# lazear/sage

Measured on AMD Instinct MI355X. Metric: spectra/sec (whole node), fragment-index search-and-score, human tryptic narrow search, higher is better.
Workload: dtype f32

## Files before the change

### include/sage_hip.h

```cpp
#ifndef SAGE_HIP_H
#define SAGE_HIP_H

#include <stddef.h>
#include <stdint.h>

#ifdef __cplusplus
extern "C" {
#endif

#define SAGE_HIP_ABI_VERSION 6

enum {
    SAGE_HIP_OK = 0,
    SAGE_HIP_ERR_INVALID = 1,
    SAGE_HIP_ERR_NO_DEVICE = 2,
    SAGE_HIP_ERR_HIP = 3,
    SAGE_HIP_ERR_UNSUPPORTED = 4,
    SAGE_HIP_ERR_OOM = 5,
    SAGE_HIP_ERR_INTERNAL = 6
};

enum { SAGE_TOL_PPM = 0, SAGE_TOL_PCT = 1, SAGE_TOL_DA = 2 };
typedef struct SageTolerance {
    int32_t kind;
// ... 143 lines not shown
    const float* precursor_mz;
    const uint8_t* precursor_charge;
    const float* isolation_lo;
    const float* isolation_hi;
    const float* scan_start_time;
    const float* inverse_ion_mobility;
    const uint32_t* file_id;
} SageRawBatch;

int sage_hip_batch_process_upload(SageScorer* scorer, const SageRawBatch* raw, uint64_t take_top_n, int deisotope,
                                  float min_deisotope_mz, uint32_t min_peaks, SageDeviceBatch** out, uint32_t* out_npeaks);
int sage_hip_batch_download(SageDeviceBatch* batch, uint64_t* peak_off, float* masses, float* intensities, float* tic);

int sage_hip_initial_hits(SageScorer* scorer, SageDeviceBatch* batch, uint64_t* packed, uint32_t cap,
                          uint32_t* len, uint64_t* matched_peaks, uint64_t* scored_candidates);

typedef struct SageFragments {
    uint64_t capacity;
    uint64_t* psm_off;
    uint8_t* kinds;
    int32_t* charges;
    int32_t* fragment_ordinals;
    float* intensities;
    float* mz_calculated;
    float* mz_experimental;
} SageFragments;
int sage_hip_annotate_resident(SageScorer* scorer, SageDeviceBatch* batch, const SageFeature* features,
                               const uint32_t* counts, SageFragments* out);

int sage_hip_quick_score_resident(SageScorer* scorer, SageDeviceBatch* batch, int prefilter_low_memory, uint8_t* keep);

typedef struct SageTiming {
    float prelim_ms;
    float rescore_ms;
    float total_ms;
    uint32_t n_launches;
    uint32_t n_wide;
    uint32_t arena_entries;
    uint32_t n_retry;
    float retry_ms;
    uint32_t n_tied;
    uint32_t n_ways;
} SageTiming;
int sage_hip_last_timing(const SageScorer* scorer, SageTiming* out);
int sage_hip_scorer_set_timing_interval(SageScorer* scorer, uint32_t every);

int sage_hip_host_alloc(uint64_t bytes, void** out);
void sage_hip_host_free(void* p);

int sage_hip_debug_phase_cycles(SageScorer* scorer, unsigned long long* out32);
int sage_hip_debug_prune_counters(SageScorer* scorer, unsigned long long* out4);
int sage_hip_debug_filter_counters(SageScorer* scorer, unsigned long long* out4);
int sage_hip_debug_heavy_counters(SageScorer* scorer, unsigned long long* out2);
int sage_hip_debug_handover_route(SageScorer* scorer, uint32_t* out);

typedef struct SageDbLayout {
    uint64_t np, nf;
    uint32_t tile_shift, n_tiles, lut_stride;
    float lut_scale;
    uint32_t tile2_shift, n_tiles2, lut2_stride;
    float lut2_scale;
    uint32_t lut2_words;
    uint32_t pep_lut_bins;
    float pep_lut_inv_w;
    uint32_t ion_lo_bits, ion_hi_bits;
    uint32_t max_ions, max_len;
    uint64_t tm2_pos_len;
} SageDbLayout;
int sage_hip_debug_db_layout(SageDeviceDb* db, SageDbLayout* out);
enum {
    SAGE_DB_IONS = 0, SAGE_DB_ION_OFF = 1, SAGE_DB_PM_OFF = 2, SAGE_DB_PEP_INFO = 3, SAGE_DB_PEP_MONO = 4, SAGE_DB_PEP_LUT = 5,
    SAGE_DB_PM_FRAG = 6, SAGE_DB_TM_FRAG = 7, SAGE_DB_TM2_FRAG = 8, SAGE_DB_TM_LUT = 9, SAGE_DB_TM2_L1 = 10, SAGE_DB_TM2_POS = 11
};
int sage_hip_debug_db_table(SageDeviceDb* db, int table, void* out, uint64_t cap_bytes, uint64_t* out_bytes);

typedef struct SageRescoreInput {
    uint64_t n;
    const SageFeature* features;
    const float* aligned_rt;
    const float* delta_rt_model;
    const float* delta_ims_model;
    SageTolerance precursor_tol;
    const uint32_t* peptide_key;
    uint32_t n_peptide_keys;
    const uint32_t* protein_key;
    uint32_t n_protein_keys;
} SageRescoreInput;

typedef struct SageRescoreOutput {
    float* discriminant_score;
    float* posterior_error;
    float* spectrum_q;
    float* peptide_q;
    float* protein_q;
    uint32_t* order;
    uint64_t passing_spectrum;
    uint64_t passing_peptide;
    uint64_t passing_protein;
    int32_t lda_fitted;
    double coef[20];
    float device_ms;
} SageRescoreOutput;

int sage_hip_rescore(int device, const SageRescoreInput* in, SageRescoreOutput* out);

typedef struct SageRtInput {
// ... 227 lines not shown
```

### sage_amd/_lib.py

```python
import ctypes as C
import os

import numpy as np

from . import build as _build

c_float_p = C.POINTER(C.c_float)
c_u8_p = C.POINTER(C.c_uint8)
c_u32_p = C.POINTER(C.c_uint32)
c_u64_p = C.POINTER(C.c_uint64)


class SageTolerance(C.Structure):
    _fields_ = [("kind", C.c_int32), ("lo", C.c_float), ("hi", C.c_float)]


class SageTheoretical(C.Structure):
    _fields_ = [("peptide_index", C.c_uint32), ("fragment_mz", C.c_float)]


class SageDbParams(C.Structure):
    _fields_ = [
        ("bucket_size", C.c_uint64),
        ("missed_cleavages", C.c_int32),
# ... 263 lines not shown
_lib = None


def lib_path():
    return _build.LIB


def load():
    global _lib
    if _lib is not None:
        return _lib
    if not os.path.exists(_build.LIB) or (os.environ.get("SAGE_HIP_REBUILD") == "1"):
        _build.build(verbose=False)
    lib = C.CDLL(_build.LIB)
    vp = C.c_void_p
    sig = {
        "sage_hip_last_error": (C.c_char_p, []),
        "sage_hip_abi_version": (C.c_int, []),
        "sage_hip_hostdb_build": (C.c_int, [C.c_char_p, C.POINTER(SageDbParams), C.POINTER(vp)]),
        "sage_hip_hostdb_free": (None, [vp]),
        "sage_hip_hostdb_view": (C.c_int, [vp, C.POINTER(SageDbView)]),
        "sage_hip_hostdb_peptide_string": (C.c_uint64, [vp, C.c_uint64, C.c_char_p, C.c_uint64]),
        "sage_hip_hostdb_peptide_proteins": (C.c_uint64, [vp, C.c_uint64, C.c_char_p, C.c_uint64]),
        "sage_hip_hostdb_peptide_info": (C.c_int, [vp, C.c_uint64, c_u32_p, c_u8_p]),
        "sage_hip_process_ms2": (C.c_uint64, [C.c_uint64, C.c_int, C.c_float, c_float_p, c_float_p, C.c_uint64,
                                              C.c_uint8, c_float_p, c_float_p, c_float_p]),
        "sage_hip_device_count": (C.c_int, []),
        "sage_hip_db_create": (C.c_int, [C.POINTER(SageDbView), C.c_int, C.POINTER(vp)]),
        "sage_hip_db_destroy": (None, [vp]),
        "sage_hip_db_device_bytes": (C.c_uint64, [vp]),
        "sage_hip_scorer_create": (C.c_int, [vp, C.POINTER(SageScorerParams), C.POINTER(vp)]),
        "sage_hip_scorer_destroy": (None, [vp]),
        "sage_hip_scorer_clone": (C.c_int, [vp, C.POINTER(vp)]),
        "sage_hip_score_batch": (C.c_int, [vp, C.POINTER(SageSpectrumBatch), vp, c_u32_p]),
        "sage_hip_batch_upload": (C.c_int, [vp, C.POINTER(SageSpectrumBatch), C.POINTER(vp)]),
        "sage_hip_batch_free": (None, [vp]),
        "sage_hip_batch_process_upload": (C.c_int, [vp, C.POINTER(SageRawBatch), C.c_uint64, C.c_int, C.c_float, C.c_uint32,
                                                    C.POINTER(vp), c_u32_p]),
        "sage_hip_batch_download": (C.c_int, [vp, c_u64_p, c_float_p, c_float_p, c_float_p]),
        "sage_hip_batch_upload_kinds": (C.c_int, [vp, C.POINTER(SageSpectrumBatch), c_u8_p, C.POINTER(vp)]),
        "sage_hip_batch_process_upload_kinds": (C.c_int, [vp, C.POINTER(SageRawBatch), c_u8_p, C.c_uint64, C.c_int, C.c_float,
                                                          C.c_uint32, C.POINTER(vp), c_u32_p]),
        "sage_hip_score_batch_kinds": (C.c_int, [vp, C.POINTER(SageSpectrumBatch), c_u8_p, vp, c_u32_p]),
        "sage_hip_score_resident": (C.c_int, [vp, vp, vp, c_u32_p]),
        "sage_hip_initial_hits": (C.c_int, [vp, vp, c_u64_p, C.c_uint32, c_u32_p, c_u64_p, c_u64_p]),
        "sage_hip_last_timing": (C.c_int, [vp, C.POINTER(SageTiming)]),
        "sage_hip_scorer_set_timing_interval": (C.c_int, [vp, C.c_uint32]),
        "sage_hip_annotate_resident": (C.c_int, [vp, vp, vp, c_u32_p, C.POINTER(SageFragments)]),
        "sage_hip_quick_score_resident": (C.c_int, [vp, vp, C.c_int, c_u8_p]),
        "sage_hip_debug_phase_cycles": (C.c_int, [vp, c_u64_p]),
        "sage_hip_debug_prune_counters": (C.c_int, [vp, c_u64_p]),
        "sage_hip_debug_filter_counters": (C.c_int, [vp, c_u64_p]),
        "sage_hip_debug_heavy_counters": (C.c_int, [vp, c_u64_p]),
        "sage_hip_debug_handover_route": (C.c_int, [vp, c_u32_p]),
        "sage_hip_debug_db_layout": (C.c_int, [vp, C.POINTER(SageDbLayout)]),
        "sage_hip_debug_db_table": (C.c_int, [vp, C.c_int, vp, C.c_uint64, c_u64_p]),
        "sage_hip_host_alloc": (C.c_int, [C.c_uint64, C.POINTER(vp)]),
        "sage_hip_host_free": (None, [vp]),
        "sage_hip_rescore": (C.c_int, [C.c_int, C.POINTER(SageRescoreInput), C.POINTER(SageRescoreOutput)]),
        "sage_hip_hostdb_competition_keys": (C.c_int, [vp, c_u32_p, C.c_uint64, c_u32_p, c_u32_p, c_u32_p, c_u32_p]),
        "sage_hip_predict_rt": (C.c_int, [C.c_int, C.POINTER(SageRtInput), C.POINTER(SageRtOutput)]),
        "sage_hip_hostdb_feature_peptides": (C.c_int, [vp, c_u32_p, C.c_uint64, c_u64_p, c_u8_p, c_float_p]),
        "sage_hip_mzml_read": (C.c_int, [C.c_char_p, C.c_uint32, C.c_int, C.POINTER(vp)]),
        "sage_hip_mzml_view": (C.c_int, [vp, C.POINTER(SageRawBatch)]),
        "sage_hip_mzml_check_searchable": (C.c_int, [vp]),
        "sage_hip_mzml_spectrum_id": (C.c_char_p, [vp, C.c_uint64]),
        "sage_hip_mzml_free": (None, [vp]),
        "sage_hip_mzml_read_sn": (C.c_int, [C.c_char_p, C.c_uint32, C.c_int, C.c_int, C.POINTER(vp)]),
        "sage_hip_mzml_ion_injection_time": (C.c_float, [vp, C.c_uint64]),
        "sage_hip_mzml_precursor_ref": (C.c_char_p, [vp, C.c_uint64]),
        "sage_hip_mgf_read": (C.c_int, [C.c_char_p, C.c_uint32, C.POINTER(vp)]),
        "sage_hip_mzml_isolation_kinds": (C.c_int, [vp, c_u8_p]),
        "sage_hip_mzml_charge_zero": (C.c_int, [vp, c_u8_p]),
        "sage_hip_parse_f32": (C.c_int, [C.c_char_p, C.c_uint64, c_float_p]),
        "sage_hip_tmt": (C.c_int, [C.c_int, C.POINTER(SageTmtInput), C.POINTER(SageTmtOutput)]),
        "sage_hip_write_tmt": (C.c_int, [C.c_char_p, C.POINTER(C.c_char_p), C.c_uint32, C.c_uint64, c_u32_p, C.POINTER(C.c_char_p),
                                         c_float_p, c_float_p, C.POINTER(C.c_char_p), C.c_uint32]),
        "sage_hip_write_results": (C.c_int, [C.c_char_p, C.c_int, vp, vp, C.c_uint64, c_u64_p, c_u64_p, C.POINTER(C.c_char_p),
                                             C.c_uint32, C.POINTER(C.c_char_p), C.POINTER(SagePostColumns)]),
        "sage_hip_write_results_grouped": (C.c_int, [C.c_char_p, C.c_int, vp, vp, C.c_uint64, c_u64_p, c_u64_p, C.POINTER(C.c_char_p),
                                                     C.c_uint32, C.POINTER(C.c_char_p), C.POINTER(SagePostColumns),
                                                     C.POINTER(SageGroupColumns)]),
        "sage_hip_protein_groups": (C.c_int, [C.c_int, vp, C.POINTER(SageGroupInput), C.POINTER(SageGroupOutput)]),
        "sage_hip_group_string": (C.c_char_p, [vp, C.c_uint64]),
        "sage_hip_group_strings_free": (None, [vp]),
        "sage_hip_group_graph_build": (C.c_int, [vp, c_u32_p, C.c_uint64, C.POINTER(vp)]),
        "sage_hip_group_graph_view": (C.c_int, [vp, C.POINTER(SageGroupGraphView)]),
        "sage_hip_group_graph_free": (None, [vp]),
        "sage_hip_hostdb_protein_name": (C.c_uint64, [vp, C.c_uint64, C.c_char_p, C.c_uint64]),
        "sage_hip_lfq": (C.c_int, [C.c_int, C.POINTER(SageLfqInput), C.POINTER(SageLfqOutput)]),
        "sage_hip_lfq_im": (C.c_int, [C.c_int, C.POINTER(SageLfqInput), C.POINTER(SageLfqMobility), C.POINTER(SageLfqOutput)]),
        "sage_hip_mzml_mobility": (c_float_p, [vp]),
        "sage_hip_mzml_has_mobility": (C.c_int, [vp, c_u8_p]),
        "sage_hip_write_lfq": (C.c_int, [C.c_char_p, vp, C.POINTER(SageLfqOutput), c_u64_p, C.c_uint64, C.POINTER(C.c_char_p),
                                         C.c_uint32]),
        "sage_hip_fasta_num_targets": (C.c_int, [C.c_char_p, C.POINTER(SageDbParams), c_u64_p]),
        "sage_hip_prefilter_chunk_size": (C.c_int, [C.c_char_p, C.POINTER(SageDbParams), C.c_uint64, c_u64_p]),
        "sage_hip_hostdb_build_chunk": (C.c_int, [C.c_char_p, C.POINTER(SageDbParams), C.c_uint64, C.c_uint64, C.POINTER(vp)]),
        "sage_hip_hostdb_merge_kept": (C.c_int, [C.POINTER(vp), C.POINTER(c_u8_p), C.c_uint32, C.POINTER(SageDbParams),
                                                 C.POINTER(vp)]),
    }
    for name, (res, args) in sig.items():
        fn = getattr(lib, name)
        fn.restype = res
        fn.argtypes = args
    _lib = lib
    return lib


EXPORTED_SYMBOLS = [
    "sage_hip_last_error", "sage_hip_abi_version", "sage_hip_hostdb_build", "sage_hip_hostdb_free",
    "sage_hip_hostdb_view", "sage_hip_hostdb_peptide_string", "sage_hip_hostdb_peptide_proteins",
    "sage_hip_hostdb_peptide_info", "sage_hip_process_ms2", "sage_hip_device_count", "sage_hip_db_create", "sage_hip_db_destroy",
    "sage_hip_db_device_bytes", "sage_hip_scorer_create", "sage_hip_scorer_destroy", "sage_hip_scorer_clone", "sage_hip_score_batch",
    "sage_hip_batch_upload", "sage_hip_batch_free", "sage_hip_batch_process_upload", "sage_hip_batch_download", "sage_hip_score_resident", "sage_hip_initial_hits",
    "sage_hip_last_timing", "sage_hip_scorer_set_timing_interval", "sage_hip_annotate_resident", "sage_hip_quick_score_resident", "sage_hip_debug_phase_cycles", "sage_hip_debug_prune_counters", "sage_hip_debug_filter_counters", "sage_hip_debug_heavy_counters", "sage_hip_debug_handover_route", "sage_hip_debug_db_layout", "sage_hip_debug_db_table", "sage_hip_host_alloc", "sage_hip_host_free",
    "sage_hip_rescore", "sage_hip_hostdb_competition_keys", "sage_hip_fasta_num_targets", "sage_hip_prefilter_chunk_size",
    "sage_hip_hostdb_build_chunk", "sage_hip_hostdb_merge_kept", "sage_hip_predict_rt", "sage_hip_hostdb_feature_peptides",
    "sage_hip_write_results", "sage_hip_mzml_read", "sage_hip_mzml_view", "sage_hip_mzml_check_searchable", "sage_hip_mzml_spectrum_id", "sage_hip_mzml_free",
    "sage_hip_lfq", "sage_hip_write_lfq", "sage_hip_mzml_read_sn", "sage_hip_mzml_ion_injection_time", "sage_hip_mzml_precursor_ref",
    "sage_hip_tmt", "sage_hip_write_tmt", "sage_hip_mgf_read", "sage_hip_mzml_isolation_kinds", "sage_hip_mzml_charge_zero",
    "sage_hip_parse_f32", "sage_hip_batch_upload_kinds", "sage_hip_batch_process_upload_kinds", "sage_hip_score_batch_kinds",
    "sage_hip_lfq_im", "sage_hip_mzml_mobility", "sage_hip_mzml_has_mobility",
    "sage_hip_protein_groups", "sage_hip_group_string", "sage_hip_group_strings_free", "sage_hip_group_graph_build",
    "sage_hip_group_graph_view", "sage_hip_group_graph_free", "sage_hip_hostdb_protein_name", "sage_hip_write_results_grouped",
]


def check(rc):
    if rc != 0:
        msg = load().sage_hip_last_error()
        raise SageHipError(f"libsage_hip status {rc}: {msg.decode() if msg else ''}")


def as_ptr(arr, ctype):
    return arr.ctypes.data_as(C.POINTER(ctype))
```

### sage_amd/csrc/capi.hip

```cpp
#include <hip/hip_runtime.h>
#include <algorithm>
#include <atomic>
#include <cmath>
#include <chrono>
#include <cstring>
#include <memory>
#include <future>
#include <mutex>
#include <string>
#include <vector>

#include "crlog.h"
#include "device_types.h"
#define HIP_FAILED(e, what) fail(status_of(e), std::string(what) + ": " + hipGetErrorString(e))
#include "hip_host.h"
#include "host_db.hpp"

using namespace sagehip;

namespace {

thread_local std::string g_last_error;

int fail(int code, const std::string& msg) {
// ... 2160 lines not shown
    HIP_TRY(hipMemcpy(st.data(), s->ws.status.p, (size_t)n * 4, hipMemcpyDeviceToHost));
    for (uint32_t i = 0; i < n; i++) {
        if (st[i] != ST_OK && st[i] != ST_OK_ORDERED) return fail(SAGE_HIP_ERR_UNSUPPORTED, "spectrum " + std::to_string(i) + ": status " + std::to_string(st[i]));
        for (uint32_t j = 0; j < len[i]; j++) packed[(size_t)i * cap + j] = c[(size_t)i * kmax + j];
        if (matched_peaks) matched_peaks[i] = tot[2 * i];
        if (scored_candidates) scored_candidates[i] = tot[2 * i + 1];
    }
    return SAGE_HIP_OK;
}

int sage_hip_debug_phase_cycles(SageScorer* s, unsigned long long* out32) {
    if (!s || !out32) return fail(SAGE_HIP_ERR_INVALID, "null argument");
    if (!s->dbg.p) return fail(SAGE_HIP_ERR_INVALID, "set SAGE_HIP_PHASE_CLOCKS=1 before creating the scorer");
    std::vector<unsigned long long> all(4096 * 32);
    HIP_TRY(hipMemcpy(all.data(), s->dbg.p, all.size() * 8, hipMemcpyDeviceToHost));
    for (int k = 0; k < 32; k++) out32[k] = 0;
    for (size_t b = 0; b < 4096; b++)
        for (int k = 0; k < 32; k++) out32[k] += all[b * 32 + k];
    return SAGE_HIP_OK;
}

int sage_hip_debug_prune_counters(SageScorer* s, unsigned long long* out4) {
    if (!s || !out4) return fail(SAGE_HIP_ERR_INVALID, "null argument");
    if (!s->dbg.p) return fail(SAGE_HIP_ERR_INVALID, "set SAGE_HIP_PHASE_CLOCKS=1 before creating the scorer");
    std::vector<unsigned long long> all((size_t)DBG_BLOCKS * DBG_PRUNE_WORDS);
    HIP_TRY(hipMemcpy(all.data(), s->dbg.p + (size_t)DBG_BLOCKS * 32, all.size() * 8, hipMemcpyDeviceToHost));
    for (uint32_t k = 0; k < 4; k++) out4[k] = 0;
    for (size_t b = 0; b < DBG_BLOCKS; b++)
        for (uint32_t k = 0; k < 4; k++) out4[k] += all[b * DBG_PRUNE_WORDS + k];
    return SAGE_HIP_OK;
}
int sage_hip_debug_filter_counters(SageScorer* s, unsigned long long* out4) {
    if (!s || !out4) return fail(SAGE_HIP_ERR_INVALID, "null argument");
    if (!s->dbg.p) return fail(SAGE_HIP_ERR_INVALID, "set SAGE_HIP_PHASE_CLOCKS=1 before creating the scorer");
    std::vector<unsigned long long> all((size_t)DBG_BLOCKS * DBG_PRUNE_WORDS);
    HIP_TRY(hipMemcpy(all.data(), s->dbg.p + (size_t)DBG_BLOCKS * 32, all.size() * 8, hipMemcpyDeviceToHost));
    for (uint32_t k = 0; k < 4; k++) out4[k] = 0;
    for (size_t b = 0; b < DBG_BLOCKS; b++)
        for (uint32_t k = 0; k < 4; k++) out4[k] += all[b * DBG_PRUNE_WORDS + 4 + k];
    return SAGE_HIP_OK;
}

int sage_hip_debug_heavy_counters(SageScorer* s, unsigned long long* out2) {
    if (!s || !out2) return fail(SAGE_HIP_ERR_INVALID, "null argument");
    if (!s->dbg.p) return fail(SAGE_HIP_ERR_INVALID, "set SAGE_HIP_PHASE_CLOCKS=1 before creating the scorer");
    std::vector<unsigned long long> all((size_t)DBG_BLOCKS * DBG_PRUNE_WORDS);
    HIP_TRY(hipMemcpy(all.data(), s->dbg.p + (size_t)DBG_BLOCKS * 32, all.size() * 8, hipMemcpyDeviceToHost));
    out2[0] = out2[1] = 0;
    for (size_t b = 0; b < DBG_BLOCKS; b++)
        for (uint32_t k = 0; k < 2; k++) out2[k] += all[b * DBG_PRUNE_WORDS + 8 + k];
    return SAGE_HIP_OK;
}

int sage_hip_debug_handover_route(SageScorer* s, uint32_t* out) {
    if (!s || !out) return fail(SAGE_HIP_ERR_INVALID, "null argument");
    *out = s->last_hand ? 1u : 0u;
    return SAGE_HIP_OK;
}

int sage_hip_debug_db_layout(SageDeviceDb* db, SageDbLayout* out) {
    if (!db || !out) return fail(SAGE_HIP_ERR_INVALID, "null argument");
    const DevDbView& v = db->view;
    std::memset(out, 0, sizeof *out);
    out->np = v.np;
    out->nf = v.nf;
    out->tile_shift = v.tile_shift;
    out->n_tiles = v.n_tiles;
    out->lut_stride = v.lut_stride;
    out->lut_scale = v.lut_scale;
    out->tile2_shift = v.tile2_shift;
    out->n_tiles2 = v.n_tiles2;
    out->lut2_stride = v.lut2_stride;
    out->lut2_scale = v.lut2_scale;
    out->lut2_words = v.lut2_words;
    out->pep_lut_bins = v.pep_lut_bins;
    out->pep_lut_inv_w = v.pep_lut_inv_w;
    out->ion_lo_bits = db->ion_lo_bits;
    out->ion_hi_bits = db->ion_hi_bits;
    out->max_ions = db->max_ions;
    out->max_len = db->max_len;
    out->tm2_pos_len = db->tm2_pos.n;
    return SAGE_HIP_OK;
}

int sage_hip_debug_db_table(SageDeviceDb* db, int table, void* out, uint64_t cap_bytes, uint64_t* out_bytes) {
    if (!db || !out_bytes) return fail(SAGE_HIP_ERR_INVALID, "null argument");
    HIP_TRY(hipSetDevice(db->device));
    if (table == SAGE_DB_PM_FRAG)
        if (int rc = ensure_pm_frag(db)) return rc;
    const void* src = nullptr;
    uint64_t bytes = 0;
    switch (table) {
        case SAGE_DB_IONS: src = db->ions.p; bytes = db->ions.bytes() - 8 * sizeof(float); break;
        case SAGE_DB_ION_OFF: src = db->ion_off.p; bytes = db->ion_off.bytes(); break;
        case SAGE_DB_PM_OFF: src = db->pm_off.p; bytes = db->pm_off.bytes(); break;
        case SAGE_DB_PEP_INFO: src = db->pep_info.p; bytes = db->pep_info.bytes(); break;
        case SAGE_DB_PEP_MONO: src = db->pep_mono.p; bytes = db->pep_mono.bytes(); break;
        case SAGE_DB_PEP_LUT: src = db->pep_lut.p; bytes = db->pep_lut.bytes(); break;
        case SAGE_DB_PM_FRAG: src = db->pm_frag.p; bytes = db->pm_frag.bytes(); break;
        case SAGE_DB_TM_FRAG: src = db->tm_frag.p; bytes = db->tm_frag.bytes(); break;
        case SAGE_DB_TM2_FRAG: src = db->tm2_frag.p; bytes = db->tm2_frag.bytes(); break;
        case SAGE_DB_TM_LUT: src = db->tm_lut.p; bytes = db->tm_lut.bytes(); break;
        case SAGE_DB_TM2_L1: src = db->tm2_l1.p; bytes = db->tm2_l1.bytes(); break;
        case SAGE_DB_TM2_POS: src = db->tm2_pos.p; bytes = db->tm2_pos.bytes(); break;
        default: return fail(SAGE_HIP_ERR_INVALID, "sage_hip_debug_db_table: unknown table id");
    }
// ... 65 lines not shown
```

### sage_amd/csrc/core.h

```cpp
#pragma once
#include <stdint.h>

#if defined(__HIPCC__)
#define SAGE_HD __host__ __device__ __forceinline__
#else
#define SAGE_HD inline
#endif

namespace sagecore {

constexpr float PROTON = 1.0072764f;
constexpr float NEUTRON = 1.00335f;

struct Tol {
    int kind;
    float lo, hi;
};

SAGE_HD void tol_bounds(const Tol& t, float center, float& out_lo, float& out_hi) {
    if (t.kind == 0) {
        float dlo = center * t.lo / 1000000.0f;
        float dhi = center * t.hi / 1000000.0f;
        out_lo = center + dlo;
        out_hi = center + dhi;
// ... 351 lines not shown
SAGE_HD void run_matched_packed(uint64_t& r, uint32_t index) {
    const uint32_t next = (uint32_t)(r & 0x1FFFFFu), length = (uint32_t)((r >> 21) & 0x1FFFFFu), longest = (uint32_t)(r >> 42);
    if ((next ? next - 1u : 0u) == index) return;
    const uint32_t nl = next == index ? length + 1u : 1u;
    r = (uint64_t)(index + 1u) | ((uint64_t)nl << 21) | ((uint64_t)(nl > longest ? nl : longest) << 42);
}
SAGE_HD uint32_t run_longest_packed(uint64_t r) { return (uint32_t)(r >> 42); }

template <uint32_t BITS, class R>
SAGE_HD void run_matched_mask_fields(R& r, uint64_t S, uint32_t idx0) {
    constexpr uint32_t FIELD = (1u << BITS) - 1u;
    if (!S) return;
    const uint32_t next = (uint32_t)r & FIELD, length = (uint32_t)(r >> BITS) & FIELD;
    uint32_t longest = (uint32_t)(r >> (2u * BITS));
    if ((next ? next - 1u : 0u) == idx0 + (uint32_t)__builtin_ctzll(S)) {
        S &= S - 1ull;
        if (!S) return;
    }
    const uint32_t t0 = (uint32_t)__builtin_ctzll(S);
    const uint64_t from_t0 = S >> t0;
    const uint32_t n0 = ~from_t0 ? (uint32_t)__builtin_ctzll(~from_t0) : 64u;
    uint32_t nl = next == idx0 + t0 ? length + n0 : n0, end = t0 + n0;
    if (nl > longest) longest = nl;
    const uint64_t rest = end >= 64u ? 0ull : S & (~0ull << end);
    if (rest) {
        uint32_t best = 0;
        for (uint64_t x = rest; x; x &= x << 1) best++;
        if (best > longest) longest = best;
        const uint32_t lz = (uint32_t)__builtin_clzll(rest);
        const uint64_t from_top = ~(rest << lz);
        nl = from_top ? (uint32_t)__builtin_clzll(from_top) : 64u;
        end = 64u - lz;
    }
    r = (R)(idx0 + end) | ((R)nl << BITS) | ((R)longest << (2u * BITS));
}
SAGE_HD void run_matched_mask(uint32_t& r, uint64_t S, uint32_t idx0) { run_matched_mask_fields<10>(r, S, idx0); }
SAGE_HD void run_matched_mask(uint64_t& r, uint64_t S, uint32_t idx0) { run_matched_mask_fields<21>(r, S, idx0); }

struct KindSeg {
    uint32_t lo, len, idx0, kind;
};
SAGE_HD KindSeg kind_seg_first(uint32_t j0, uint32_t lm1) {
    KindSeg g = {0u, 0u, j0, 0u};
    while (g.idx0 >= lm1) { g.idx0 -= lm1; g.kind++; }
    g.len = lm1 - g.idx0 < 64u ? lm1 - g.idx0 : 64u;
    return g;
}
SAGE_HD KindSeg kind_seg_next(const KindSeg& g, uint32_t lm1) {
    const uint32_t lo = g.lo + g.len;
    const uint32_t len = lm1 < 64u - lo ? lm1 : 64u - lo;
    return KindSeg{lo, len, 0u, g.kind + 1u};
}
SAGE_HD uint64_t kind_seg_mask(const KindSeg& g) { return g.len >= 64u ? ~0ull : ((1ull << g.len) - 1ull) << (g.lo & 63u); }

struct Score {
    uint32_t peptide;
    uint32_t matched_b, matched_y;
    float summed_b, summed_y;
    uint32_t longest_b, longest_y;
    float ppm_difference;
    uint32_t precursor_charge;
    int isotope_error;
};

SAGE_HD void score_candidate(Score& s, const float* ions, uint32_t lm1, const uint8_t* ion_kinds, uint32_t n_kinds,
                             uint32_t max_fc, const float* masses, const float* intensities, uint32_t n_peaks,
                             const Tol& fragment_tol) {
    Run b_run = {0, 0, 0, 0}, y_run = {0, 0, 0, 0};
    s.matched_b = s.matched_y = 0;
    s.summed_b = s.summed_y = 0.0f;
    s.ppm_difference = 0.0f;
    for (uint32_t k = 0; k < n_kinds; k++) {
        const bool nterm_kind = ion_kinds[k] <= 2;
        const float* series = ions + (uint64_t)k * lm1;
        for (uint32_t idx = 0; idx < lm1; idx++) {
            const float frag = series[idx];
            for (uint32_t charge = 1; charge < max_fc; charge++) {
                const float mz = frag / (float)charge;
                const int pk = select_most_intense_peak(masses, intensities, n_peaks, mz, fragment_tol);
                if (pk < 0) continue;
                const float peak_mass = masses[pk];
                const float peak_intensity = intensities[pk];
                const float d = __builtin_fabsf(mz - peak_mass);
                s.ppm_difference += peak_intensity * d * 2E6f / (mz + peak_mass);
                if (nterm_kind) {
                    s.matched_b += 1;
                    s.summed_b += peak_intensity;
                    run_matched(b_run, idx);
                } else {
                    s.matched_y += 1;
                    s.summed_y += peak_intensity;
                    run_matched(y_run, idx);
                }
            }
        }
    }
    s.longest_b = b_run.longest;
    s.longest_y = y_run.longest;
    s.ppm_difference /= s.summed_b + s.summed_y;
}

SAGE_HD void lut_cells(float lo, float hi, float scale, uint32_t stride, uint32_t& icl, uint32_t& ich) {
    float cl = __builtin_floorf(lo * scale);
    float ch = __builtin_floorf(hi * scale) + 1.0f;
    cl = cl > 0.0f ? cl : 0.0f;
    ch = ch > 0.0f ? ch : 0.0f;
// ... 148 lines not shown
```

### sage_amd/csrc/device_types.h

```cpp
#pragma once
#include <stdint.h>

#include <string>

#include "../../include/sage_hip.h"
#include "core.h"

namespace sagehip {

struct DevDbView {
    const float* pep_mono;
    uint32_t np;
    const uint32_t* pep_lut;
    uint32_t pep_lut_bins;
    float pep_lut_inv_w;
    const SageTheoretical* pm_frag;
    const uint64_t* pm_off;
    const float* ions;
    const uint64_t* ion_off;
    const uint32_t* pep_info;
    const SageTheoretical* tm_frag;
    const uint32_t* tm_lut;
    uint32_t tile_shift;
    uint32_t n_tiles;
    uint32_t lut_stride;
    float lut_scale;
    const SageTheoretical* tm2_frag;
    const sagecore::LutWord* tm2_l1;
    const uint32_t* tm2_pos;
    uint32_t lut2_words;
    uint32_t tile2_shift;
    uint32_t n_tiles2;
    uint32_t lut2_stride;
    float lut2_scale;
    uint64_t nf;
    uint8_t ion_kinds[8];
    uint32_t n_kinds;
};

constexpr uint32_t TILE_SHIFT_MAX = 15;
__host__ __device__ inline size_t tm_lut_index(uint32_t t, uint32_t c, uint32_t lut_stride) { return (size_t)t * lut_stride + c; }

constexpr uint32_t DBG_BLOCKS = 4096, DBG_PRUNE_WORDS = 10;
constexpr size_t DBG_TOTAL_WORDS = (size_t)DBG_BLOCKS * (32 + DBG_PRUNE_WORDS);

struct DevScorer {
    sagecore::Tol precursor_tol, fragment_tol;
    sagecore::PbmReach pbm_reach;
    uint32_t min_matched_peaks;
    int min_isotope_err, max_isotope_err;
    uint32_t min_precursor_charge, max_precursor_charge;
    uint32_t override_precursor_charge;
    int max_fragment_charge;
    uint32_t chimera;
    uint32_t report_psms;
    uint32_t wide_window;
    int score_type;
    uint32_t kmax;
    uint32_t big_path;
    uint32_t long_runs;
    uint32_t tol_mode;
    uint32_t list_cap;
    uint32_t wcap;
    uint32_t dbg_flags;
    uint32_t prune_min;
    uint32_t rescore_general;
    uint32_t xcd_chunk;
    uint32_t fast_log;
    uint32_t exact;
};

struct DevBatchView {
    uint32_t n;
    const uint32_t* n_dev;
    uint32_t spec_base;
    const uint64_t* peak_off;
    const float* masses;
    const float* intensities;
    const float* precursor_mz;
    const uint8_t* precursor_charge;
    const float* isolation_lo;
    const float* isolation_hi;
    const float* tic;
    const float* rt;
    const float* ims;
    const uint32_t* file_id;
    const uint32_t* order;
    uint32_t probe;
    uint32_t pcap;
    uint32_t fzcap;
    const uint4* sched;
    const uint8_t* iso_kind;
    uint32_t sched_stride;
    uint32_t sched_win;
    const struct WindowKey* sched_key;
};
// ... 156 lines not shown
```

### sage_amd/csrc/kernels.hip

```cpp
#include <hip/hip_runtime.h>

#include <type_traits>

#include "crlog.h"
#include "device_types.h"

using namespace sagecore;

namespace sagehip {

namespace {

#ifndef SAGE_PRELIM_WAVES
#define SAGE_PRELIM_WAVES 5
#endif
#ifndef SAGE_RESCORE_WAVES
#define SAGE_RESCORE_WAVES 5
#endif
#ifndef SAGE_NARROW_WAVES
#define SAGE_NARROW_WAVES 5
#endif
#ifndef SAGE_PROBE_PER_LANE
#define SAGE_PROBE_PER_LANE 2
#endif
#ifndef SAGE_PROBE_CELLS
#define SAGE_PROBE_CELLS 4
#endif
#ifndef SAGE_TILE8_CELLS
#define SAGE_TILE8_CELLS 2
#endif
#ifndef SAGE_MARK_BLOCKS8
#define SAGE_MARK_BLOCKS8 96
#endif
#ifndef SAGE_MARK_BLOCKS16
#define SAGE_MARK_BLOCKS16 40
#endif
#ifndef SAGE_COOP_MIN_HITS
#define SAGE_COOP_MIN_HITS 12
#endif
#ifndef SAGE_COOP_MAX_LANES
#define SAGE_COOP_MAX_LANES 2
#endif
#ifndef SAGE_CNT_MODE
#define SAGE_CNT_MODE 0
#endif
#ifndef SAGE_SCAN_SKIP
#define SAGE_SCAN_SKIP 1
#endif
#if SAGE_NARROW_WAVES
#define SAGE_NARROW_WAVES_ATTR __attribute__((amdgpu_waves_per_eu(SAGE_NARROW_WAVES, SAGE_NARROW_WAVES)))
#else
#define SAGE_NARROW_WAVES_ATTR
#endif
#if SAGE_PRELIM_WAVES
#define SAGE_PRELIM_WAVES_ATTR __attribute__((amdgpu_waves_per_eu(SAGE_PRELIM_WAVES, SAGE_PRELIM_WAVES)))
#else
#define SAGE_PRELIM_WAVES_ATTR
#endif
#if SAGE_RESCORE_WAVES
#define SAGE_RESCORE_WAVES_ATTR __attribute__((amdgpu_waves_per_eu(SAGE_RESCORE_WAVES, SAGE_RESCORE_WAVES)))
#else
#define SAGE_RESCORE_WAVES_ATTR
#endif

constexpr uint32_t WAVE = 64;
constexpr uint32_t NO_WINDOW = 0xFFFFFFFFu;
constexpr uint32_t FAST_TIE_WORDS = PBM_WORDS + PLUT_BINS;
constexpr uint32_t CNT_ROW_HEADER = 4;
constexpr uint32_t PROBE_BATCH_WORDS = SAGE_PROBE_PER_LANE * 64;
constexpr uint32_t PROBE_TCS_WORDS = PROBE_BATCH_WORDS <= 64 ? 64 : PROBE_BATCH_WORDS <= 128 ? 128 : PROBE_BATCH_WORDS <= 256 ? 256 : 512;
constexpr uint32_t PROBE_TABLE_WORDS = 4 * PROBE_BATCH_WORDS + PROBE_TCS_WORDS;

enum { DBG_PRUNE_CAND = 0, DBG_PRUNE_ITEMS = 1, DBG_PRUNE_EARLY = 2, DBG_PRUNE_MIXED = 3 };
enum { DBG_FILTER_FLAT_CHUNKS = 4, DBG_FILTER_FLAT_TRIPS = 5, DBG_FILTER_FLAT_WOULD = 6, DBG_FILTER_LANE_TRIPS = 7 };
enum { DBG_HEAVY_CHUNKS = 8, DBG_HEAVY_ITEMS = 9 };
enum { DBG_NARROW_LUT = 26, DBG_NARROW_CELLS = 27, DBG_RESCORE = 28, DBG_TILE_LUT = 29, DBG_TILE_CELLS = 30, DBG_TILE_CAND = 31 };
struct PhaseClock {
    unsigned long long* slot;
    long long t;
    __device__ __forceinline__ void bytes(int which, unsigned long long n) {
        if (slot) atomicAdd(&slot[which - row_base], n);
    }
    int row_base;
    unsigned long long* prune;
    uint32_t pruned_here;
    __device__ __forceinline__ void pruned(uint64_t lanes, uint32_t items) {
        if (slot && lanes) {
            pruned_here += (uint32_t)__popcll(lanes);
            if ((threadIdx.x & 63u) == 0) {
                atomicAdd(&prune[DBG_PRUNE_CAND], (unsigned long long)__popcll(lanes));
                atomicAdd(&prune[DBG_PRUNE_ITEMS], (unsigned long long)items);
            }
        }
    }
    __device__ __forceinline__ void filter_trips(bool flat, uint32_t flat_trips, uint32_t lane_trips) {
        if (slot && (threadIdx.x & 63u) == 0) {
            if (flat) {
                atomicAdd(&prune[DBG_FILTER_FLAT_CHUNKS], 1ull);
                atomicAdd(&prune[DBG_FILTER_FLAT_TRIPS], (unsigned long long)flat_trips);
                atomicAdd(&prune[DBG_FILTER_FLAT_WOULD], (unsigned long long)lane_trips);
            } else {
                atomicAdd(&prune[DBG_FILTER_LANE_TRIPS], (unsigned long long)lane_trips);
            }
        }
    }
    __device__ __forceinline__ void heavy(uint32_t items) {
        if (slot && (threadIdx.x & 63u) == 0) {
            atomicAdd(&prune[DBG_HEAVY_CHUNKS], 1ull);
            atomicAdd(&prune[DBG_HEAVY_ITEMS], (unsigned long long)items);
        }
    }
    __device__ __forceinline__ void prune_outcome(bool left_early, bool any_pass) {
        if (slot && (threadIdx.x & 63u) == 0) {
            if (left_early) atomicAdd(&prune[DBG_PRUNE_EARLY], 1ull);
            else if (any_pass && pruned_here) atomicAdd(&prune[DBG_PRUNE_MIXED], 1ull);
        }
        pruned_here = 0;
    }
    __device__ __forceinline__ void start(unsigned long long* dbg, uint32_t blk, uint32_t kernel) {
        slot = dbg ? dbg + (size_t)(blk % DBG_BLOCKS) * 32 + kernel * 8 : nullptr;
        row_base = (int)kernel * 8;
        prune = dbg ? dbg + (size_t)DBG_BLOCKS * 32 + (size_t)(blk % DBG_BLOCKS) * DBG_PRUNE_WORDS : nullptr;
        pruned_here = 0;
        if (slot) t = clock64();
    }
    __device__ __forceinline__ void mark(int phase) {
        if (slot) {
            const long long n = clock64();
            if ((threadIdx.x & 63u) == 0) atomicAdd(&slot[phase], (unsigned long long)(n - t));
            t = n;
        }
    }
    __device__ __forceinline__ void rebase(uint32_t kernel) {
        if (slot) slot += (int)kernel * 8 - row_base;
        row_base = (int)kernel * 8;
    }
};

struct NoClock {
    static constexpr unsigned long long* slot = nullptr;
    __device__ __forceinline__ void bytes(int, unsigned long long) {}
    __device__ __forceinline__ void pruned(uint64_t, uint32_t) {}
    __device__ __forceinline__ void prune_outcome(bool, bool) {}
    __device__ __forceinline__ void filter_trips(bool, uint32_t, uint32_t) {}
    __device__ __forceinline__ void heavy(uint32_t) {}
    __device__ __forceinline__ void start(unsigned long long*, uint32_t, uint32_t) {}
    __device__ __forceinline__ void mark(int) {}
    __device__ __forceinline__ void rebase(uint32_t) {}
};

__device__ __forceinline__ uint32_t lane_id() { return threadIdx.x & 63u; }

constexpr uint32_t N_XCD = 8;
__device__ __forceinline__ uint32_t xcd_position_fwd(uint32_t b, uint32_t n, uint32_t chunk) {
    if (chunk == 0) return b;
    const uint32_t group = N_XCD * chunk;
    if (b >= n / group * group) return b;
    const uint32_t x = b % N_XCD, i = b / N_XCD;
    return ((i / chunk) * N_XCD + x) * chunk + i % chunk;
}
__device__ __forceinline__ uint32_t xcd_position(uint32_t b, uint32_t n, uint32_t chunk) {
    const uint32_t p = xcd_position_fwd(b, n, chunk & 0x7FFFFFFFu);
    return (chunk & 0x80000000u) ? n - 1 - p : p;
}

__device__ __forceinline__ uint32_t fresh_zero() {
    uint32_t z;
    asm volatile("v_mov_b32 %0, 0" : "=v"(z));
    return z;
}
__device__ __forceinline__ uint32_t uni(uint32_t v) { return (uint32_t)__builtin_amdgcn_readfirstlane((int)v); }
__device__ __forceinline__ float unif(float v) { return __int_as_float(__builtin_amdgcn_readfirstlane(__float_as_int(v))); }
__device__ __forceinline__ uint64_t uni64(uint64_t v) { return ((uint64_t)uni((uint32_t)(v >> 32)) << 32) | uni((uint32_t)v); }

__device__ __forceinline__ uint32_t wave_sum_dpp(uint32_t v) {
    v += (uint32_t)__builtin_amdgcn_update_dpp(0, (int)v, 0xb1, 0xf, 0xf, false);
    v += (uint32_t)__builtin_amdgcn_update_dpp(0, (int)v, 0x4e, 0xf, 0xf, false);
    v += (uint32_t)__builtin_amdgcn_update_dpp(0, (int)v, 0x124, 0xf, 0xf, false);
    v += (uint32_t)__builtin_amdgcn_update_dpp(0, (int)v, 0x128, 0xf, 0xf, false);
    v += (uint32_t)__builtin_amdgcn_update_dpp(0, (int)v, 0x142, 0xf, 0xf, false);
    v += (uint32_t)__builtin_amdgcn_update_dpp(0, (int)v, 0x143, 0xf, 0xf, false);
    return (uint32_t)__builtin_amdgcn_readlane((int)v, 63);
}

__device__ __forceinline__ uint32_t wave_incl_scan_dpp(uint32_t v) {
    v += (uint32_t)__builtin_amdgcn_update_dpp(0, (int)v, 0x111, 0xf, 0xf, true);
    v += (uint32_t)__builtin_amdgcn_update_dpp(0, (int)v, 0x112, 0xf, 0xf, true);
    v += (uint32_t)__builtin_amdgcn_update_dpp(0, (int)v, 0x114, 0xf, 0xf, true);
    v += (uint32_t)__builtin_amdgcn_update_dpp(0, (int)v, 0x118, 0xf, 0xf, true);
    v += (uint32_t)__builtin_amdgcn_update_dpp(0, (int)v, 0x142, 0xa, 0xf, false);
    v += (uint32_t)__builtin_amdgcn_update_dpp(0, (int)v, 0x143, 0xc, 0xf, false);
    return v;
}

__device__ __forceinline__ uint32_t wave_incl_scan_max_dpp(uint32_t v) {
#define SAGE_SMAX(CTRL, ROWS, BC)                                                                  \
    {                                                                                              \
        const uint32_t t = (uint32_t)__builtin_amdgcn_update_dpp(0, (int)v, CTRL, ROWS, 0xf, BC);  \
// ... 2448 lines not shown
                    if (any_fz3 && nfz >= 3u) {
                        const uint32_t* const wp = (const uint32_t*)(a3 + at);
                        const uint32_t w0 = wp[0], w1 = wp[1], w2 = wp[2];
                        m3 = (uint64_t)flat_mask_word(w0, w1, start) | ((uint64_t)flat_mask_word(w1, w2, start) << 32);
                    }
                }
            }
            flat_trips = (T + 63u) / 64u;
        }
        if (pc.slot) {
            uint32_t would = act ? (n_here + 3u) >> 2 : 0u;
            for (int o = 32; o; o >>= 1) { const uint32_t v = (uint32_t)__shfl_xor((int)would, o, 64); would = v > would ? v : would; }
            pc.filter_trips(flat, flat_trips, would);
        }
        if (act && !flat) {
            const float* __restrict__ q = my + j0;
            float n0 = q[0], n1 = q[1], n2 = q[2], n3 = q[3];
            for (uint32_t r = 0; r < n_here; r += 4) {
                const float i0 = n0, i1 = n1, i2 = n2, i3 = n3;
                n0 = q[r + 4]; n1 = q[r + 5]; n2 = q[r + 6]; n3 = q[r + 7];
                const uint32_t x0 = pbm_index(i0), x1 = pbm_index(i1), x2 = pbm_index(i2), x3 = pbm_index(i3);
                const uint32_t t1 = pbm_bit(x0) | (pbm_bit(x1) << 1) | (pbm_bit(x2) << 2) | (pbm_bit(x3) << 3);
                m1 |= (uint64_t)t1 << r;
                if (any_fz2) {
                    const uint32_t t2 = pbm_bit(x0 >> 1) | (pbm_bit(x1 >> 1) << 1) | (pbm_bit(x2 >> 1) << 2) | (pbm_bit(x3 >> 1) << 3);
                    m2 |= (uint64_t)t2 << r;
                }
                if (any_fz3) {
                    const uint32_t t3 = pbm_bit(__umulhi(x0, 0xAAAAAAABu) >> 1) | (pbm_bit(__umulhi(x1, 0xAAAAAAABu) >> 1) << 1) |
                                        (pbm_bit(__umulhi(x2, 0xAAAAAAABu) >> 1) << 2) | (pbm_bit(__umulhi(x3, 0xAAAAAAABu) >> 1) << 3);
                    m3 |= (uint64_t)t3 << r;
                }
            }
        }
        if (act) {
            const uint64_t in_chunk = n_here >= 64u ? ~0ull : (1ull << n_here) - 1ull;
            m1 &= in_chunk;
            m2 = nfz >= 2 ? m2 & in_chunk : 0ull;
            m3 = nfz >= 3 ? m3 & in_chunk : 0ull;
            if (nfz > 3) m1 = m2 = m3 = in_chunk;
        }
        pc.mark(6);
        uint32_t hc = act && nfz <= 3 ? (uint32_t)(__popcll(m1) + __popcll(m2) + __popcll(m3)) : 0u;
        {
            const bool drop = hc != 0u && j0 + 64u >= nions && (mm & 0xFFFFu) + (mm >> 16) + hc < sc.prune_min;
            if (pc.slot) pc.pruned(__ballot(drop), wave_sum(drop ? hc : 0u));
            if (drop) {
                m1 = m2 = m3 = 0ull;
                hc = 0u;
            }
        }
        uint64_t bigs = (sc.dbg_flags & 32u) ? 0ull : __ballot(hc > ((sc.dbg_flags & 32768u) ? 0u : COOP_MIN_HITS));
        if ((uint32_t)__popcll(bigs) > COOP_MAX_LANES && !(sc.dbg_flags & 64u)) bigs = 0ull;
        while (bigs) {
            const uint32_t L = (uint32_t)__ffsll((long long)bigs) - 1;
            bigs &= bigs - 1;
            const uint64_t M1 = lane_value(m1, L), M2 = lane_value(m2, L), M3 = lane_value(m3, L);
            const uint64_t base_L = lane_value((uint64_t)ion_base, L);
            const uint32_t lm1_L = (uint32_t)__builtin_amdgcn_readlane((int)lm1, (int)L);
            const bool on1 = (M1 >> lane) & 1ull, on2 = (M2 >> lane) & 1ull, on3 = (M3 >> lane) & 1ull;
            float it1 = 0.f, it2 = 0.f, it3 = 0.f, tm1 = 0.f, tm2 = 0.f, tm3 = 0.f;
            bool ok1 = false, ok2 = false, ok3 = false;
            if (on1 || on2 || on3) {
                const float ionv = db.ions[base_L + j0 + lane];
#define SAGE_COOP_LOOKUP(C, ON, OK, IT, TM)                                                              \
    if (ON) {                                                                                            \
        const float mz = fragment_mz<FAST>(ionv, (C));                                                   \
        float flo, fhi;                                                                                  \
        tol_bounds_mode<FAST>(sc.fragment_tol, sym_tol, mz, flo, fhi);                                   \
        const int pk = select_peak_lut(pm, pi, P, plut, inv_w, flo, fhi);                                \
        if (pk >= 0) {                                                                                   \
const float peak_mass = pm[pk], peak_intensity = pi[pk];                                     \
OK = true;                                                                                   \
IT = peak_intensity;                                                                         \
TM = peak_intensity * __builtin_fabsf(mz - peak_mass) * 2E6f / (mz + peak_mass);             \
        }                                                                                                \
    }
                SAGE_COOP_LOOKUP(1, on1, ok1, it1, tm1)
                SAGE_COOP_LOOKUP(2, on2, ok2, it2, tm2)
                SAGE_COOP_LOOKUP(3, on3, ok3, it3, tm3)
#undef SAGE_COOP_LOOKUP
            }
            const uint64_t K1 = __ballot(ok1), K2 = __ballot(ok2), K3 = __ballot(ok3);
            float u_sb = lane_valuef(s.summed_b, L), u_sy = lane_valuef(s.summed_y, L), u_pp = lane_valuef(s.ppm_difference, L);
            uint32_t u_mm = (uint32_t)__builtin_amdgcn_readlane((int)mm, (int)L);
            RunReg u_b = lane_run(b_run, L);
            RunReg u_y = lane_run(y_run, L);
            uint64_t anyK = K1 | K2 | K3;
            if (pc.slot) pc.heavy((uint32_t)(__popcll(K1) + __popcll(K2) + __popcll(K3)));
            for (KindSeg g = kind_seg_first(j0, lm1_L); anyK && g.lo < 64u; g = kind_seg_next(g, lm1_L)) {
                const uint64_t seg = kind_seg_mask(g);
                uint64_t S = anyK & seg;
                if (!S) continue;
                anyK ^= S;
                const bool nterm = (nterm_mask >> g.kind) & 1u;
                u_mm += (uint32_t)(__popcll(K1 & seg) + __popcll(K2 & seg) + __popcll(K3 & seg)) << (nterm ? 0u : 16u);
                if (nterm) run_matched_mask(u_b, S >> g.lo, g.idx0);
                else run_matched_mask(u_y, S >> g.lo, g.idx0);
                float acc = nterm ? u_sb : u_sy;
                do {
                    const uint32_t bit = (uint32_t)__builtin_ctzll(S);
                    S &= S - 1ull;
                    if ((K1 >> bit) & 1ull) { acc += lane_valuef(it1, bit); u_pp += lane_valuef(tm1, bit); }
                    if ((K2 >> bit) & 1ull) { acc += lane_valuef(it2, bit); u_pp += lane_valuef(tm2, bit); }
                    if ((K3 >> bit) & 1ull) { acc += lane_valuef(it3, bit); u_pp += lane_valuef(tm3, bit); }
                } while (S);
                if (nterm) u_sb = acc;
                else u_sy = acc;
            }
            if (lane == L) {
                s.summed_b = u_sb; s.summed_y = u_sy; s.ppm_difference = u_pp;
                mm = u_mm;
                b_run = u_b; y_run = u_y;
                m1 = m2 = m3 = 0ull;
            }
        }
        pc.mark(7);
        if (DENSE && dense_ok && !(sc.dbg_flags & 128u) && __ballot(j0 + 64u < nions) == 0ull && __ballot(act && nfz > 3u) == 0ull) {
            const uint32_t hcnt = act ? (uint32_t)(__popcll(m1) + __popcll(m2) + __popcll(m3)) : 0u;
            const uint32_t incl = wave_incl_scan_dpp(hcnt);
            const uint32_t T = (uint32_t)__builtin_amdgcn_readlane((int)incl, 63);
            if (T == 0u) continue;
            if (T <= ((sc.dbg_flags & 256u) ? 64u : DENSE_CAP)) {
                uint32_t* const dW = (uint32_t*)pbm;
                float* const dB = (float*)(dW + DENSE_CAP);
                uint16_t* const dT = (uint16_t*)(dB + DENSE_CAP);
                uint32_t* const dF = (uint32_t*)(dT + DENSE_CAP);
                uint32_t pos = incl - hcnt;
                uint64_t any = m1 | m2 | m3;
                while (any) {
                    const uint32_t bit = (uint32_t)__ffsll((long long)any) - 1;
                    any &= any - 1;
                    uint32_t kind_i = 0, idx = j0 + bit;
                    while (idx >= lm1) { idx -= lm1; kind_i++; }
                    const uint32_t word = idx | (((nterm_mask >> kind_i) & 1u) << 15) | (bit << 16) | (lane << 24);
                    if ((m1 >> bit) & 1ull) dW[pos++] = word | (1u << 22);
                    if (any_fz2 && ((m2 >> bit) & 1ull)) dW[pos++] = word | (2u << 22);
                    if (any_fz3 && ((m3 >> bit) & 1ull)) dW[pos++] = word | (3u << 22);
                }
                lds_sync();
                for (uint32_t base = 0; base < T; base += WAVE) {
                    const uint32_t i = base + lane;
                    const uint32_t word = i < T ? dW[i] : 0u;
                    const uint32_t src = (word >> 24) << 2;
                    const uint64_t ib = ((uint64_t)(uint32_t)__builtin_amdgcn_ds_bpermute((int)src, (int)(uint32_t)(ion_base >> 32)) << 32) |
                                        (uint32_t)__builtin_amdgcn_ds_bpermute((int)src, (int)(uint32_t)ion_base);
                    bool ok = false;
                    if (i < T) {
                        const float ionv = db.ions[ib + j0 + ((word >> 16) & 63u)];
                        const uint32_t c = (word >> 22) & 3u;
                        float mz = c == 2u ? ionv * 0.5f : ionv;
// ... 1278 lines not shown
```

Baseline: 155.6 million.

## Compact cooperative heavy-lane lookups into one wave trip via LDS

For heavy lanes in the dense flat path, the per-charge lookups are packed into a single list in LDS using mbcnt prefix positions, so every item is handled in one pass across the wave instead of up to three sequential per-charge passes. Intensities and ppm terms are written to LDS and reduced by three lanes with float4 reads, which replaces the serial per-bit readlane accumulation loop. This adds several LDS barriers and changes the order of float summation, which can shift results slightly. A debug counter that records which route each heavy lane takes is also added.

```diff
diff --git a/include/sage_hip.h b/include/sage_hip.h
--- a/include/sage_hip.h
+++ b/include/sage_hip.h
@@ -219,6 +219,7 @@
 int sage_hip_debug_prune_counters(SageScorer* scorer, unsigned long long* out4);
 int sage_hip_debug_filter_counters(SageScorer* scorer, unsigned long long* out4);
 int sage_hip_debug_heavy_counters(SageScorer* scorer, unsigned long long* out2);
+int sage_hip_debug_heavy_routes(SageScorer* scorer, unsigned long long* out2);
 int sage_hip_debug_handover_route(SageScorer* scorer, uint32_t* out);
 
 typedef struct SageDbLayout {
diff --git a/sage_amd/_lib.py b/sage_amd/_lib.py
--- a/sage_amd/_lib.py
+++ b/sage_amd/_lib.py
@@ -339,6 +339,7 @@
         "sage_hip_debug_prune_counters": (C.c_int, [vp, c_u64_p]),
         "sage_hip_debug_filter_counters": (C.c_int, [vp, c_u64_p]),
         "sage_hip_debug_heavy_counters": (C.c_int, [vp, c_u64_p]),
+        "sage_hip_debug_heavy_routes": (C.c_int, [vp, c_u64_p]),
         "sage_hip_debug_handover_route": (C.c_int, [vp, c_u32_p]),
         "sage_hip_debug_db_layout": (C.c_int, [vp, C.POINTER(SageDbLayout)]),
         "sage_hip_debug_db_table": (C.c_int, [vp, C.c_int, vp, C.c_uint64, c_u64_p]),
@@ -401,7 +402,7 @@
     "sage_hip_hostdb_peptide_info", "sage_hip_process_ms2", "sage_hip_device_count", "sage_hip_db_create", "sage_hip_db_destroy",
     "sage_hip_db_device_bytes", "sage_hip_scorer_create", "sage_hip_scorer_destroy", "sage_hip_scorer_clone", "sage_hip_score_batch",
     "sage_hip_batch_upload", "sage_hip_batch_free", "sage_hip_batch_process_upload", "sage_hip_batch_download", "sage_hip_score_resident", "sage_hip_initial_hits",
-    "sage_hip_last_timing", "sage_hip_scorer_set_timing_interval", "sage_hip_annotate_resident", "sage_hip_quick_score_resident", "sage_hip_debug_phase_cycles", "sage_hip_debug_prune_counters", "sage_hip_debug_filter_counters", "sage_hip_debug_heavy_counters", "sage_hip_debug_handover_route", "sage_hip_debug_db_layout", "sage_hip_debug_db_table", "sage_hip_host_alloc", "sage_hip_host_free",
+    "sage_hip_last_timing", "sage_hip_scorer_set_timing_interval", "sage_hip_annotate_resident", "sage_hip_quick_score_resident", "sage_hip_debug_phase_cycles", "sage_hip_debug_prune_counters", "sage_hip_debug_filter_counters", "sage_hip_debug_heavy_counters", "sage_hip_debug_heavy_routes", "sage_hip_debug_handover_route", "sage_hip_debug_db_layout", "sage_hip_debug_db_table", "sage_hip_host_alloc", "sage_hip_host_free",
     "sage_hip_rescore", "sage_hip_hostdb_competition_keys", "sage_hip_fasta_num_targets", "sage_hip_prefilter_chunk_size",
     "sage_hip_hostdb_build_chunk", "sage_hip_hostdb_merge_kept", "sage_hip_predict_rt", "sage_hip_hostdb_feature_peptides",
     "sage_hip_write_results", "sage_hip_mzml_read", "sage_hip_mzml_view", "sage_hip_mzml_check_searchable", "sage_hip_mzml_spectrum_id", "sage_hip_mzml_free",
diff --git a/sage_amd/csrc/capi.hip b/sage_amd/csrc/capi.hip
--- a/sage_amd/csrc/capi.hip
+++ b/sage_amd/csrc/capi.hip
@@ -2236,6 +2236,17 @@
     return SAGE_HIP_OK;
 }
 
+int sage_hip_debug_heavy_routes(SageScorer* s, unsigned long long* out2) {
+    if (!s || !out2) return fail(SAGE_HIP_ERR_INVALID, "null argument");
+    if (!s->dbg.p) return fail(SAGE_HIP_ERR_INVALID, "set SAGE_HIP_PHASE_CLOCKS=1 before creating the scorer");
+    std::vector<unsigned long long> all((size_t)DBG_BLOCKS * DBG_PRUNE_WORDS);
+    HIP_TRY(hipMemcpy(all.data(), s->dbg.p + (size_t)DBG_BLOCKS * 32, all.size() * 8, hipMemcpyDeviceToHost));
+    out2[0] = out2[1] = 0;
+    for (size_t b = 0; b < DBG_BLOCKS; b++)
+        for (uint32_t k = 0; k < 2; k++) out2[k] += all[b * DBG_PRUNE_WORDS + 10 + k];
+    return SAGE_HIP_OK;
+}
+
 int sage_hip_debug_handover_route(SageScorer* s, uint32_t* out) {
     if (!s || !out) return fail(SAGE_HIP_ERR_INVALID, "null argument");
     *out = s->last_hand ? 1u : 0u;
diff --git a/sage_amd/csrc/core.h b/sage_amd/csrc/core.h
--- a/sage_amd/csrc/core.h
+++ b/sage_amd/csrc/core.h
@@ -427,6 +427,15 @@
     return KindSeg{lo, len, 0u, g.kind + 1u};
 }
 SAGE_HD uint64_t kind_seg_mask(const KindSeg& g) { return g.len >= 64u ? ~0ull : ((1ull << g.len) - 1ull) << (g.lo & 63u); }
+
+constexpr uint32_t COOP_ITEMS_CAP = 64;
+SAGE_HD uint32_t coop_items_below(uint64_t M1, uint64_t M2, uint64_t M3, uint32_t i) {
+    const uint64_t below = i >= 64u ? ~0ull : (1ull << i) - 1ull;
+    return (uint32_t)(__builtin_popcountll(M1 & below) + __builtin_popcountll(M2 & below) + __builtin_popcountll(M3 & below));
+}
+SAGE_HD uint32_t coop_item_pos(uint64_t M1, uint64_t M2, uint64_t M3, uint32_t i, uint32_t c) {
+    return coop_items_below(M1, M2, M3, i) + (c >= 2u ? (uint32_t)((M1 >> i) & 1ull) : 0u) + (c >= 3u ? (uint32_t)((M2 >> i) & 1ull) : 0u);
+}
 
 struct Score {
     uint32_t peptide;
diff --git a/sage_amd/csrc/device_types.h b/sage_amd/csrc/device_types.h
--- a/sage_amd/csrc/device_types.h
+++ b/sage_amd/csrc/device_types.h
@@ -41,7 +41,7 @@
 constexpr uint32_t TILE_SHIFT_MAX = 15;
 __host__ __device__ inline size_t tm_lut_index(uint32_t t, uint32_t c, uint32_t lut_stride) { return (size_t)t * lut_stride + c; }
 
-constexpr uint32_t DBG_BLOCKS = 4096, DBG_PRUNE_WORDS = 10;
+constexpr uint32_t DBG_BLOCKS = 4096, DBG_PRUNE_WORDS = 12;
 constexpr size_t DBG_TOTAL_WORDS = (size_t)DBG_BLOCKS * (32 + DBG_PRUNE_WORDS);
 
 struct DevScorer {
diff --git a/sage_amd/csrc/kernels.hip b/sage_amd/csrc/kernels.hip
--- a/sage_amd/csrc/kernels.hip
+++ b/sage_amd/csrc/kernels.hip
@@ -74,6 +74,7 @@
 enum { DBG_PRUNE_CAND = 0, DBG_PRUNE_ITEMS = 1, DBG_PRUNE_EARLY = 2, DBG_PRUNE_MIXED = 3 };
 enum { DBG_FILTER_FLAT_CHUNKS = 4, DBG_FILTER_FLAT_TRIPS = 5, DBG_FILTER_FLAT_WOULD = 6, DBG_FILTER_LANE_TRIPS = 7 };
 enum { DBG_HEAVY_CHUNKS = 8, DBG_HEAVY_ITEMS = 9 };
+enum { DBG_HEAVY_ONE_TRIP = 10, DBG_HEAVY_PER_CHARGE = 11 };
 enum { DBG_NARROW_LUT = 26, DBG_NARROW_CELLS = 27, DBG_RESCORE = 28, DBG_TILE_LUT = 29, DBG_TILE_CELLS = 30, DBG_TILE_CAND = 31 };
 struct PhaseClock {
     unsigned long long* slot;
@@ -110,6 +111,9 @@
             atomicAdd(&prune[DBG_HEAVY_ITEMS], (unsigned long long)items);
         }
     }
+    __device__ __forceinline__ void heavy_route(bool one_trip) {
+        if (slot && (threadIdx.x & 63u) == 0) atomicAdd(&prune[one_trip ? DBG_HEAVY_ONE_TRIP : DBG_HEAVY_PER_CHARGE], 1ull);
+    }
     __device__ __forceinline__ void prune_outcome(bool left_early, bool any_pass) {
         if (slot && (threadIdx.x & 63u) == 0) {
             if (left_early) atomicAdd(&prune[DBG_PRUNE_EARLY], 1ull);
@@ -144,6 +148,7 @@
     __device__ __forceinline__ void prune_outcome(bool, bool) {}
     __device__ __forceinline__ void filter_trips(bool, uint32_t, uint32_t) {}
     __device__ __forceinline__ void heavy(uint32_t) {}
+    __device__ __forceinline__ void heavy_route(bool) {}
     __device__ __forceinline__ void start(unsigned long long*, uint32_t, uint32_t) {}
     __device__ __forceinline__ void mark(int) {}
     __device__ __forceinline__ void rebase(uint32_t) {}
@@ -2698,6 +2703,7 @@
         }
         uint64_t bigs = (sc.dbg_flags & 32u) ? 0ull : __ballot(hc > ((sc.dbg_flags & 32768u) ? 0u : COOP_MIN_HITS));
         if ((uint32_t)__popcll(bigs) > COOP_MAX_LANES && !(sc.dbg_flags & 64u)) bigs = 0ull;
+        const bool coop_lds = FLAT && DENSE && dense_ok && !(sc.dbg_flags & 262144u) && __ballot(j0 + 64u < nions) == 0ull;
         while (bigs) {
             const uint32_t L = (uint32_t)__ffsll((long long)bigs) - 1;
             bigs &= bigs - 1;
@@ -2707,7 +2713,77 @@
             const bool on1 = (M1 >> lane) & 1ull, on2 = (M2 >> lane) & 1ull, on3 = (M3 >> lane) & 1ull;
             float it1 = 0.f, it2 = 0.f, it3 = 0.f, tm1 = 0.f, tm2 = 0.f, tm3 = 0.f;
             bool ok1 = false, ok2 = false, ok3 = false;
-            if (on1 || on2 || on3) {
+            const uint32_t N = (uint32_t)(__popcll(M1) + __popcll(M2) + __popcll(M3));
+            const bool one_trip = coop_lds && N <= COOP_ITEMS_CAP;
+            if (pc.slot) pc.heavy_route(one_trip);
+            float sum_b = 0.f, sum_y = 0.f, sum_p = 0.f;
+            if (one_trip) {
+                uint32_t* const cD = (uint32_t*)pbm;
+                float* const cS = (float*)(cD + 64);
+                float ionv = 0.f;
+                if (on1 || on2 || on3) ionv = db.ions[base_L + j0 + lane];
+                uint64_t NT = 0ull;
+                {
+                    uint64_t rem = M1 | M2 | M3;
+                    for (KindSeg g = kind_seg_first(j0, lm1_L); rem && g.lo < 64u; g = kind_seg_next(g, lm1_L)) {
+                        const uint64_t seg = kind_seg_mask(g);
+                        rem &= ~seg;
+                        if ((nterm_mask >> g.kind) & 1u) NT |= seg;
+                    }
+                }
+                uint32_t p1 = __builtin_amdgcn_mbcnt_hi((uint32_t)(M1 >> 32), __builtin_amdgcn_mbcnt_lo((uint32_t)M1, 0u));
+                p1 = __builtin_amdgcn_mbcnt_hi((uint32_t)(M2 >> 32), __builtin_amdgcn_mbcnt_lo((uint32_t)M2, p1));
+                p1 = __builtin_amdgcn_mbcnt_hi((uint32_t)(M3 >> 32), __builtin_amdgcn_mbcnt_lo((uint32_t)M3, p1));
+                const uint32_t p2 = p1 + (on1 ? 1u : 0u), p3 = p2 + (on2 ? 1u : 0u);
+                const uint32_t dsc = lane | ((uint32_t)((NT >> lane) & 1ull) << 8);
+                lds_sync();
+                if (on1) cD[p1] = dsc | (1u << 16);
+                if (on2) cD[p2] = dsc | (2u << 16);
+                if (on3) cD[p3] = dsc | (3u << 16);
+                lds_sync();
+                const uint32_t item = lane < N ? cD[lane] : 0u;
+                const float iv = __uint_as_float((uint32_t)__builtin_amdgcn_ds_bpermute((int)((item & 63u) << 2), (int)__float_as_uint(ionv)));
+                float sb = 0.f, sy = 0.f, st = 0.f;
+                bool ok = false;
+                if (lane < N) {
+                    const uint32_t c = item >> 16;
+                    float mz = c == 2u ? iv * 0.5f : iv;
+                    if (any_fz3 && c == 3u) mz = fragment_mz<FAST>(iv, 3u);
+                    float flo, fhi;
+                    tol_bounds_mode<FAST>(sc.fragment_tol, sym_tol, mz, flo, fhi);
+                    const int pk = select_peak_lut(pm, pi, P, plut, inv_w, flo, fhi);
+                    if (pk >= 0) {
+                        const float peak_mass = pm[pk], peak_intensity = pi[pk];
+                        ok = true;
+                        if (item & 0x100u) sb = peak_intensity;
+                        else sy = peak_intensity;
+                        st = peak_intensity * __builtin_fabsf(mz - peak_mass) * 2E6f / (mz + peak_mass);
+                    }
+                }
+                cS[lane] = sb;
+                cS[64u + lane] = sy;
+                cS[128u + lane] = st;
+                const uint64_t Kp = __ballot(ok);
+                ok1 = on1 && ((Kp >> (p1 & 63u)) & 1ull);
+                ok2 = on2 && ((Kp >> (p2 & 63u)) & 1ull);
+                ok3 = on3 && ((Kp >> (p3 & 63u)) & 1ull);
+                lds_sync();
+                float acc = lane == 0u ? lane_valuef(s.summed_b, L) : lane == 1u ? lane_valuef(s.summed_y, L) : lane_valuef(s.ppm_difference, L);
+                if (lane < 3u) {
+                    const float4* const a = (const float4*)(cS + 64u * lane);
+                    float4 v = a[0];
+                    for (uint32_t q = 4u; q < N; q += 4u) {
+                        const float4 nv = a[q >> 2];
+                        acc += v.x; acc += v.y; acc += v.z; acc += v.w;
+                        v = nv;
+                    }
+                    acc += v.x; acc += v.y; acc += v.z; acc += v.w;
+                }
+                sum_b = lane_valuef(acc, 0u);
+                sum_y = lane_valuef(acc, 1u);
+                sum_p = lane_valuef(acc, 2u);
+                lds_sync();
+            } else if (on1 || on2 || on3) {
                 const float ionv = db.ions[base_L + j0 + lane];
 #define SAGE_COOP_LOOKUP(C, ON, OK, IT, TM)                                                              \
     if (ON) {                                                                                            \
@@ -2728,7 +2804,8 @@
 #undef SAGE_COOP_LOOKUP
             }
             const uint64_t K1 = __ballot(ok1), K2 = __ballot(ok2), K3 = __ballot(ok3);
-            float u_sb = lane_valuef(s.summed_b, L), u_sy = lane_valuef(s.summed_y, L), u_pp = lane_valuef(s.ppm_difference, L);
+            float u_sb = sum_b, u_sy = sum_y, u_pp = sum_p;
+            if (!one_trip) { u_sb = lane_valuef(s.summed_b, L); u_sy = lane_valuef(s.summed_y, L); u_pp = lane_valuef(s.ppm_difference, L); }
             uint32_t u_mm = (uint32_t)__builtin_amdgcn_readlane((int)mm, (int)L);
             RunReg u_b = lane_run(b_run, L);
             RunReg u_y = lane_run(y_run, L);
@@ -2743,6 +2820,7 @@
                 u_mm += (uint32_t)(__popcll(K1 & seg) + __popcll(K2 & seg) + __popcll(K3 & seg)) << (nterm ? 0u : 16u);
                 if (nterm) run_matched_mask(u_b, S >> g.lo, g.idx0);
                 else run_matched_mask(u_y, S >> g.lo, g.idx0);
+                if (one_trip) continue;
                 float acc = nterm ? u_sb : u_sy;
                 do {
                     const uint32_t bit = (uint32_t)__builtin_ctzll(S);
```

Result: faster. 157.7 million (median of 6 runs) (+1.3%).
